# vressegu/sdeflow-light

Hardware: AMD Instinct MI355X
Metric: score-matching train steps/sec (+ reverse-SDE sample steps/sec) (higher is better)
Workload: dtype f32

## Files before the change

sdeflow_light_amd/csrc/conv_kernels.hip:

```cpp
#include "common.h"
#include <algorithm>
#include <type_traits>
#include <stdlib.h>

#define CONV_MAX_SRC 2

struct ConvGeom {
  int N, Hi, Wi, Ho, Wo;
  int KH, KW, strideH, padH, strideW, padW;
  int mode;
  int ups;
};

struct ConvArgs {
  ConvGeom g;
  const float* src[CONV_MAX_SRC];
  int C[CONV_MAX_SRC];
  int koff[CONV_MAX_SRC];
  int nsrc;
  const float* Wp;
  int Cout, CoutP, Ktot;
  const float* bias;
  const float* samp_bias;
  int n_bias, n_samp;
// ... 601 lines not shown
#pragma unroll
          for (int c = 0; c < 2; ++c) a[c] = *reinterpret_cast<const f32x4*>(wp + c * co_stride);
#pragma unroll
          for (int r = 0; r < 4; ++r)
#pragma unroll
            for (int c = 0; c < 2; ++c)
#pragma unroll
              for (int pt = 0; pt < 2; ++pt) acc[cls][c][pt] = mfma16(a[c][r], b[pt][r], acc[cls][c][pt]);
        }
      }
    }
  }
  asm volatile("s_nop 15\n\ts_nop 7" ::: "memory");
  __builtin_amdgcn_sched_barrier(0);
#pragma unroll
  for (int c = 0; c < 2; ++c) {
    const int co = co0 + 16 * c + 4 * q;
    const f32x4 add = conv_addend(A, n, co, true);
    f32x4 cs = {0.f, 0.f, 0.f, 0.f}, css = cs;
#pragma unroll
    for (int pt = 0; pt < 2; ++pt) {
      const int yy = y0 + 2 * w + pt, xx = x0 + il;
      if (yy >= g.Hi || xx >= g.Wi) continue;
#pragma unroll
      for (int cls = 0; cls < 4; ++cls) {
        const size_t m = ((size_t)n * g.Ho + 2 * yy + (cls >> 1)) * g.Wo + 2 * xx + (cls & 1);
        conv_store_quad(A, A.out + m * A.Cout + co, acc[cls][c][pt] + add, true, co, cs, css);
      }
    }
  }
}

#define C1_LP 36
template <int PT, int KG, int EXTRA>
__global__ void __launch_bounds__(256) k_conv1x1(ConvArgs A, int P , long Mtot, int ct_per) {
  constexpr bool LDS_OUT = PT == 4;
  __shared__ __attribute__((aligned(16))) float c1_lds[4][LDS_OUT ? 16 * PT * C1_LP : 4];
  const int tid = threadIdx.x, w = tid >> 6, lane = tid & 63, il = lane & 15, q = lane >> 4;
  const long m0 = ((long)blockIdx.x * 4 + w) * (16 * PT);
  if (m0 >= Mtot) return;
  float* wl = c1_lds[w];
  const int n = __builtin_amdgcn_readfirstlane((int)(m0 / P));
  const int g0 = A.C[0] >> 4;
  const int ctot = A.C[0] + (A.nsrc > 1 ? A.C[1] : 0);
  f32x4 b[PT][KG];
#pragma unroll
  for (int pt = 0; pt < PT; ++pt) {
    const long m = m0 + 16 * pt + il;
#pragma unroll
    for (int g = 0; g < KG; ++g) {
      const bool second = g >= g0;
      const int c = (second ? 16 * (g - g0) : 16 * g) + 4 * q;
      const int C = second ? A.C[1] : A.C[0];
      b[pt][g] = *reinterpret_cast<const f32x4*>((second ? A.src[1] : A.src[0]) + (size_t)m * C + c);
    }
  }
  if (A.in_scale) {
#pragma unroll
    for (int g = 0; g < KG; ++g) {
      const bool second = g >= g0;
      const size_t o = (size_t)n * ctot + (second ? A.C[0] + 16 * (g - g0) : 16 * g) + 4 * q;
      const f32x4 ga = *reinterpret_cast<const f32x4*>(A.in_scale + o), gb = *reinterpret_cast<const f32x4*>(A.in_shift + o);
#pragma unroll
      for (int pt = 0; pt < PT; ++pt) {
        f32x4 v = b[pt][g] * ga + gb;
        if (A.in_act == 1) {
#pragma unroll
          for (int r = 0; r < 4; ++r) v[r] = v[r] * __builtin_amdgcn_rcpf(1.0f + __expf(-v[r]));
        }
        b[pt][g] = v;
      }
    }
  }
  const int ct0 = blockIdx.y * ct_per, ntile = min(A.Cout >> 4, ct0 + ct_per);
  const float* wrow = A.Wp + (size_t)il * A.Ktot + 4 * q;
  const size_t tile_stride = (size_t)16 * A.Ktot;
  constexpr int D = (KG % 4 == 0) ? 4 : 2;
  static_assert(KG % D == 0 && D <= KG, "ring slots must line up from one tile to the next");
  f32x4 an[D];
#pragma unroll
  for (int d = 0; d < D; ++d) an[d] = *reinterpret_cast<const f32x4*>(wrow + (size_t)ct0 * tile_stride + 16 * d);
  const bool has_b = A.bias && n < A.n_bias, has_s = A.samp_bias && n < A.n_samp;
  const float fb = has_b ? 1.f : 0.f, fs = has_s ? 1.f : 0.f;
  const float* bp = has_b ? A.bias + 4 * q : A.Wp;
  const float* sp = has_s ? A.samp_bias + (size_t)n * A.Cout + 4 * q : A.Wp;
  const int bstep = has_b ? 16 : 0, sstep = has_s ? 16 : 0;
  f32x4 add_n = *reinterpret_cast<const f32x4*>(bp + (size_t)ct0 * bstep) * fb + *reinterpret_cast<const f32x4*>(sp + (size_t)ct0 * sstep) * fs;
  const float* ex = EXTRA ? (A.residual ? A.residual : A.out) : nullptr;
  const size_t orow = (size_t)(m0 + il) * A.Cout + 4 * q;
  const size_t ptstep = (size_t)16 * A.Cout;
  f32x4 ex_n[EXTRA ? PT : 1];
  if (EXTRA) {
#pragma unroll
    for (int pt = 0; pt < PT; ++pt) ex_n[pt] = *reinterpret_cast<const f32x4*>(ex + orow + pt * ptstep + 16 * ct0);
  }
  for (int ct = ct0; ct < ntile; ++ct) {
    const int ctn = min(ct + 1, ntile - 1);
    f32x4 acc[PT];
#pragma unroll
    for (int pt = 0; pt < PT; ++pt) acc[pt] = f32x4{0, 0, 0, 0};
    const f32x4 add = add_n;
    f32x4 exv[EXTRA ? PT : 1];
    if (EXTRA) {
#pragma unroll
      for (int pt = 0; pt < PT; ++pt) exv[pt] = ex_n[pt];
    }
#pragma unroll
    for (int g = 0; g < KG; ++g) {
      const f32x4 a = an[g % D];
      const int ng = (g + D < KG) ? g + D : g + D - KG, nct = (g + D < KG) ? ct : ctn;
      an[g % D] = *reinterpret_cast<const f32x4*>(wrow + (size_t)nct * tile_stride + 16 * ng);
      if (g == 0) {
        add_n = *reinterpret_cast<const f32x4*>(bp + (size_t)ctn * bstep) * fb + *reinterpret_cast<const f32x4*>(sp + (size_t)ctn * sstep) * fs;
        if (EXTRA) {
#pragma unroll
          for (int pt = 0; pt < PT; ++pt) ex_n[pt] = *reinterpret_cast<const f32x4*>(ex + orow + pt * ptstep + 16 * ctn);
        }
      }
      __builtin_amdgcn_sched_barrier(0);
#pragma unroll
      for (int r = 0; r < 4; ++r)
#pragma unroll
        for (int pt = 0; pt < PT; ++pt) acc[pt] = mfma16(a[r], b[pt][g][r], acc[pt]);
    }
    f32x4 cs = {0.f, 0.f, 0.f, 0.f}, css = {0.f, 0.f, 0.f, 0.f};
    const int half = (ct - ct0) & 1;
    const bool paired = LDS_OUT && (half == 1 || ct + 1 < ntile);
#pragma unroll
    for (int pt = 0; pt < PT; ++pt) {
      f32x4 v = acc[pt] + add;
      if (EXTRA) v += exv[pt];
      if (paired) *reinterpret_cast<f32x4*>(wl + (16 * pt + il) * C1_LP + 16 * half + 4 * q) = v;
      else *reinterpret_cast<f32x4*>(A.out + orow + pt * ptstep + 16 * ct) = v;
      cs += v; css += v * v;
    }
    if (LDS_OUT && half == 1) {
      const size_t obase = (size_t)m0 * A.Cout + 16 * (ct - 1) + 4 * (lane & 7);
#pragma unroll
      for (int j = 0; j < 2 * PT; ++j) {
        const int px = 8 * j + (lane >> 3);
        const f32x4 v = *reinterpret_cast<const f32x4*>(wl + px * C1_LP + 4 * (lane & 7));
        *reinterpret_cast<f32x4*>(A.out + obase + (size_t)px * A.Cout) = v;
        if (j & 1) __builtin_amdgcn_sched_barrier(0);
      }
    }
    if (A.cstat) cstat_store(A, n, (int)((m0 % P) / (16 * PT)), 16 * ct + 4 * q, cs, css, il);
  }
}

constexpr int H18_HW = 18, H18_ITEMS = H18_HW * H18_HW * (CT_KC / 4), H18_NST = (H18_ITEMS + 255) / 256;
__device__ __forceinline__ void halo18_load(const ConvArgs& A, const ConvGeom& g, const float* src, int C, int up, int c0, size_t aff0, int n, int y0, int x0,
                                            int tid, f32x4 (&st)[H18_NST], unsigned& valid, f32x4& ga, f32x4& gb) {
  const float* base = src + (size_t)n * g.Hi * g.Wi * C;
  const int cq = c0 + 4 * (tid & 7);
  ga = f32x4{1.f, 1.f, 1.f, 1.f}; gb = f32x4{0.f, 0.f, 0.f, 0.f};
  if (A.in_scale && cq < C) {
    const size_t o = aff0 + cq;
    ga = *reinterpret_cast<const f32x4*>(A.in_scale + o);
    gb = *reinterpret_cast<const f32x4*>(A.in_shift + o);
  }
  valid = 0;
#pragma unroll
  for (int k = 0; k < H18_NST; ++k) {
    const int idx = tid + 256 * k;
    f32x4 v = {0, 0, 0, 0};
    if (idx < H18_ITEMS) {
      const int hp = idx >> 3, hy = hp / H18_HW, hx = hp - hy * H18_HW;
      const int iy = y0 + hy - 1, ix = x0 + hx - 1;
      const int c = c0 + 4 * (idx & 7);
      if (iy >= 0 && iy < (g.Hi << up) && ix >= 0 && ix < (g.Wi << up) && c < C) {
        v = *reinterpret_cast<const f32x4*>(base + ((size_t)(iy >> up) * g.Wi + (ix >> up)) * C + c);
        valid |= 1u << k;
      }
    }
    st[k] = v;
  }
}
__device__ __forceinline__ void halo18_store(const ConvArgs& A, float* buf, int tid, f32x4 (&st)[H18_NST], unsigned valid, f32x4 ga, f32x4 gb) {
  if (A.in_scale) {
// ... 132 lines not shown
__device__ __forceinline__ void wino_patch_load(f32x4 (&d)[4][4], const float* __restrict__ p00, bool last_in_row) {
#pragma unroll
  for (int i = 0; i < 4; ++i) {
    d[i][0] = *reinterpret_cast<const f32x4*>(p00 + (i * HW_ + 0) * CT_P);
    d[i][1] = *reinterpret_cast<const f32x4*>(p00 + (i * HW_ + 1) * CT_P);
  }
#pragma unroll
  for (int i = 0; i < 4; ++i)
#pragma unroll
    for (int j = 0; j < 2; ++j)
#pragma unroll
      for (int r = 0; r < 4; ++r) d[i][2 + j][r] = dpp_from_next_lane(d[i][j][r]);
  if (last_in_row) {
#pragma unroll
    for (int i = 0; i < 4; ++i) {
      d[i][2] = *reinterpret_cast<const f32x4*>(p00 + (i * HW_ + 2) * CT_P);
      d[i][3] = *reinterpret_cast<const f32x4*>(p00 + (i * HW_ + 3) * CT_P);
    }
  }
}

__device__ __forceinline__ void wino_input_transform(f32x4 (&d)[4][4]) {
#pragma unroll
  for (int j = 0; j < 4; ++j) {
    const f32x4 r0 = d[0][j] - d[2][j], r1 = d[1][j] + d[2][j], r2 = d[2][j] - d[1][j], r3 = d[1][j] - d[3][j];
    d[0][j] = r0; d[1][j] = r1; d[2][j] = r2; d[3][j] = r3;
  }
#pragma unroll
  for (int i = 0; i < 4; ++i) {
    const f32x4 c0_ = d[i][0] - d[i][2], c1_ = d[i][1] + d[i][2], c2_ = d[i][2] - d[i][1], c3_ = d[i][1] - d[i][3];
    d[i][0] = c0_; d[i][1] = c1_; d[i][2] = c2_; d[i][3] = c3_;
  }
}
__device__ __forceinline__ void wino_wfill(const float* src, float* dst, int w, size_t pos_stride, size_t a_co_stride) {
#pragma unroll
  for (int j = 0; j < 4; ++j) {
    const int pw = 4 * w + j;
    __builtin_amdgcn_global_load_lds((const __attribute__((address_space(1))) void*)(src + (size_t)(pw >> 1) * pos_stride + (pw & 1) * a_co_stride),
                                     (__attribute__((address_space(3))) void*)(dst + pw * 256), 16, 0, 0);
  }
}
template <int NPOS>
__device__ __forceinline__ void wino_mfma_lds(f32x4 (&acc)[16][2], const f32x4 (&d)[4][4], const float* wb, int pos0) {
  f32x4 a0 = *reinterpret_cast<const f32x4*>(wb), a1 = *reinterpret_cast<const f32x4*>(wb + 256);
#pragma unroll
  for (int pl = 0; pl < NPOS; ++pl) {
    const f32x4 x0 = a0, x1 = a1;
    if (pl < NPOS - 1) {
      a0 = *reinterpret_cast<const f32x4*>(wb + (2 * pl + 2) * 256);
      a1 = *reinterpret_cast<const f32x4*>(wb + (2 * pl + 3) * 256);
    }
    const int pos = pos0 + pl;
    const f32x4 b = d[pos >> 2][pos & 3];
#pragma unroll
    for (int r = 0; r < 4; ++r) {
      acc[pos][0] = mfma16(x0[r], b[r], acc[pos][0]);
      acc[pos][1] = mfma16(x1[r], b[r], acc[pos][1]);
    }
    __builtin_amdgcn_sched_barrier(0);
  }
}

template <int NCO>
__device__ __forceinline__ void wino_output_transform(const f32x4 (&acc)[16][NCO], int c, f32x4 (&Y)[4]) {
  f32x4 t0[4], t1[4];
#pragma unroll
  for (int nu = 0; nu < 4; ++nu) {
    t0[nu] = acc[nu][c] + acc[4 + nu][c] + acc[8 + nu][c];
    t1[nu] = acc[4 + nu][c] - acc[8 + nu][c] - acc[12 + nu][c];
  }
// ... 266 lines not shown
  asm volatile("s_waitcnt vmcnt(0) lgkmcnt(0)\n\ts_barrier" ::: "memory");
  float* cur = hb0;
  float* nxt = hb1;
  const int ngrp = (C + 15) >> 4;
  for (; t < n_tiles; t += gridDim.x) {
    const int tn = t + gridDim.x;
    const bool more = tn < n_tiles;
    if (more) stage_load(tn);
    f32x4 acc[16][NCO];
#pragma unroll
    for (int p = 0; p < 16; ++p)
#pragma unroll
      for (int c = 0; c < NCO; ++c) acc[p][c] = f32x4{0, 0, 0, 0};
    for (int grp = 0; grp < ngrp; ++grp) {
      f32x4 d[4][4];
#pragma unroll
      for (int i = 0; i < 4; ++i)
#pragma unroll
        for (int j = 0; j < 4; ++j) d[i][j] = *reinterpret_cast<const f32x4*>(cur + pbase + (i * HW + j) * CT_P + 16 * grp);
      wino_input_transform(d);
      wino_mfma_lds<16>(acc, d, wbuf + grp * (16 * 2 * 256) + lane * 4, 0);
    }
    int n, y0, x0;
    tile_origin<16, 16>(t, tiles_x, tiles_y, n, y0, x0);
    wino_epilogue<NCO>(A, acc, n, y0, x0, w, 0, (t - n * tiles_x * tiles_y) * 4 + w, lane);
    if (more) halo18_store(A, nxt, tid, st, valid, ga, gb);
    asm volatile("s_waitcnt lgkmcnt(0)\n\ts_barrier" ::: "memory");
    float* sw = cur; cur = nxt; nxt = sw;
  }
}

constexpr int WP_HPIECES = 21;
constexpr int WP_HSTAGE = WP_HPIECES * 64 * 4;
constexpr int WP_LDS_BYTES = (2 * 4096 + 2 * WP_HSTAGE) * (int)sizeof(float);

__global__ void __launch_bounds__(256, 2) k_conv_wino_pipe(ConvArgs A, int tiles_x, int tiles_y, int n_tiles, int n_cob) {
  extern __shared__ __attribute__((aligned(16))) float cw_lds[];
  constexpr int NCO = 2, HW = 18;
  const int tid = threadIdx.x, lane = tid & 63, il = lane & 15, q = lane >> 4;
  const int w = __builtin_amdgcn_readfirstlane(tid >> 6);
  const ConvGeom g = A.g;
  float* wbuf = cw_lds;
  float* hbuf = cw_lds + 2 * 4096;
  const int xcd = blockIdx.x & 7, loc_stride = gridDim.x >> 3;
  int loc = blockIdx.x >> 3;
  int tile = (loc / n_cob) * 8 + xcd, cob = loc % n_cob;
  if (tile >= n_tiles) return;
  const int ngrp = A.Ktot >> 4, tpi = tiles_x * tiles_y, up = g.ups ? 1 : 0;
  const size_t a_co_stride = (size_t)16 * A.Ktot, pos_stride = (size_t)A.CoutP * A.Ktot;
  const int tt = 16 * w + il, ty = tt >> 3, tx = tt & 7;
  const int P0 = 2 * ty * HW + 2 * tx, h0 = (P0 >> 1) & 3;

  auto wfill = [&](int cob_, int grp_, int half) __attribute__((always_inline)) {
    wino_wfill(A.Wp + (size_t)(cob_ * (NCO * 16) + il) * A.Ktot + 16 * grp_ + 4 * q + (size_t)(8 * half) * pos_stride,
               wbuf + half * 4096, w, pos_stride, a_co_stride);
  };
  const int Hu = g.Hi << up, Wu = g.Wi << up;
  int hpk[(WP_HPIECES + 3) / 4];
#pragma unroll
  for (int j = 0; j < (WP_HPIECES + 3) / 4; ++j) {
    const int sl = 64 * (w + 4 * j) + lane, P = sl >> 2, c = (sl & 3) ^ ((P >> 1) & 3), hy = P / HW, hx = P - hy * HW;
    hpk[j] = P < HW * HW ? (hy << 16) | (hx << 2) | c : 0x7fff << 16;
  }
  auto hfill = [&](int tile_, int grp_, int b) __attribute__((always_inline)) {
    const int n = tile_ / tpi, r = tile_ - n * tpi, ty_i = r / tiles_x, y0 = ty_i * 16, x0 = (r - ty_i * tiles_x) * 16;
    const bool s1 = 16 * grp_ >= A.C[0];
    const int C = s1 ? A.C[1] : A.C[0];
    const float* base = (s1 ? A.src[1] : A.src[0]) + (size_t)n * g.Hi * g.Wi * C + (16 * grp_ - (s1 ? A.C[0] : 0));
#pragma unroll
    for (int j = 0; j < (WP_HPIECES + 3) / 4; ++j) {
      const int m = w + 4 * j;
      if (m < WP_HPIECES) {
        int pk = hpk[j];
        asm volatile("" : "+v"(pk));
        const int c = pk & 3, iy = y0 + (pk >> 16) - 1, ix = x0 + ((pk >> 2) & 31) - 1;
        const bool in = (unsigned)iy < (unsigned)Hu && (unsigned)ix < (unsigned)Wu;
        const float* p = in ? base + (((iy >> up) * g.Wi + (ix >> up)) * C + 4 * c) : g_wino_zero;
        __builtin_amdgcn_global_load_lds((const __attribute__((address_space(1))) void*)p,
                                         (__attribute__((address_space(3))) void*)(hbuf + b * WP_HSTAGE + m * 256), 16, 0, 0);
      }
    }
  };

  f32x4 acc[16][NCO];
#pragma unroll
  for (int p = 0; p < 16; ++p)
#pragma unroll
    for (int c = 0; c < NCO; ++c) acc[p][c] = f32x4{0, 0, 0, 0};
  int grp = 0, hb = 0;
  wfill(cob, 0, 0);
  hfill(tile, 0, 0);
  for (;;) {
    int nloc = loc, ntile = tile, ncob = cob, ngrp_ = grp + 1;
    if (ngrp_ == ngrp) {
      ngrp_ = 0; nloc = loc + loc_stride;
      ntile = (nloc / n_cob) * 8 + xcd; ncob = nloc % n_cob;
    }
    const bool more = ntile < n_tiles;
    f32x4 d[4][4];
#pragma unroll
    for (int half = 0; half < 2; ++half) {
      if (half == 1 && more) asm volatile("s_waitcnt vmcnt(5) lgkmcnt(0)\n\ts_barrier" ::: "memory");
      else asm volatile("s_waitcnt vmcnt(0) lgkmcnt(0)\n\ts_barrier" ::: "memory");
      if (half == 0) {
        wfill(cob, grp, 1);
        if (more) hfill(ntile, ngrp_, hb ^ 1);
      } else if (more) {
        wfill(ncob, ngrp_, 0);
      }
      if (half == 0) {
        const float* hs = hbuf + hb * WP_HSTAGE;
#pragma unroll
        for (int i = 0; i < 4; ++i) {
          const float* rp = hs + 16 * (P0 + i * HW) + 4 * (q ^ ((h0 + i) & 3));
          d[i][0] = *reinterpret_cast<const f32x4*>(rp);
          d[i][1] = *reinterpret_cast<const f32x4*>(rp + 16);
        }
#pragma unroll
        for (int i = 0; i < 4; ++i)
#pragma unroll
          for (int j = 0; j < 2; ++j)
#pragma unroll
            for (int r = 0; r < 4; ++r) d[i][2 + j][r] = dpp_from_next_lane(d[i][j][r]);
        if (tx == 7) {
#pragma unroll
          for (int i = 0; i < 4; ++i) {
            const float* rp = hs + 16 * (P0 + i * HW + 2) + 4 * (q ^ ((h0 + i + 1) & 3));
            d[i][2] = *reinterpret_cast<const f32x4*>(rp);
            d[i][3] = *reinterpret_cast<const f32x4*>(rp + 16);
          }
        }
        wino_input_transform(d);
      }
      const float* wb = wbuf + half * 4096 + lane * 4;
      f32x4 a0 = *reinterpret_cast<const f32x4*>(wb), a1 = *reinterpret_cast<const f32x4*>(wb + 256);
#pragma unroll
      for (int pl = 0; pl < 8; ++pl) {
        const f32x4 x0_ = a0, x1_ = a1;
        if (pl < 7) {
          a0 = *reinterpret_cast<const f32x4*>(wb + (2 * pl + 2) * 256);
          a1 = *reinterpret_cast<const f32x4*>(wb + (2 * pl + 3) * 256);
        }
        const int pos = 8 * half + pl;
        const f32x4 b = d[pos >> 2][pos & 3];
#pragma unroll
        for (int r = 0; r < 4; ++r) {
          acc[pos][0] = mfma16(x0_[r], b[r], acc[pos][0]);
          acc[pos][1] = mfma16(x1_[r], b[r], acc[pos][1]);
        }
        __builtin_amdgcn_sched_barrier(0);
      }
    }
    if (ngrp_ == 0) {
      const int n = tile / tpi, r = tile - n * tpi, ty_i = r / tiles_x;
      wino_epilogue<NCO>(A, acc, n, ty_i * 16, (r - ty_i * tiles_x) * 16, w, cob * (NCO * 16), r * 4 + w, lane);
      if (!more) break;
#pragma unroll
      for (int p = 0; p < 16; ++p)
#pragma unroll
        for (int c = 0; c < NCO; ++c) acc[p][c] = f32x4{0, 0, 0, 0};
    }
    loc = nloc; tile = ntile; cob = ncob; grp = ngrp_; hb ^= 1;
  }
}

__global__ void __launch_bounds__(256) k_wino_pack_batched(const msgm_pack_job_t* __restrict__ jobs) {
  const msgm_pack_job_t J = jobs[blockIdx.y];
  const int64_t tot = (int64_t)J.rows * J.ncols;
  for (int64_t e = blockIdx.x * (int64_t)blockDim.x + threadIdx.x; e < tot; e += (int64_t)gridDim.x * blockDim.x) {
    const int c = (int)(e % J.ncols), r = (int)(e / J.ncols);
    const float* w = J.W + r * J.sr + (J.col_off + c) * J.sc;
    float gk[3][3], h[4][3];
#pragma unroll
    for (int t = 0; t < 9; ++t) gk[t / 3][t % 3] = w[t * J.st];
#pragma unroll
    for (int j = 0; j < 3; ++j) {
      h[0][j] = gk[0][j];
      h[1][j] = 0.5f * (gk[0][j] + gk[1][j] + gk[2][j]);
      h[2][j] = 0.5f * (gk[0][j] - gk[1][j] + gk[2][j]);
      h[3][j] = gk[2][j];
    }
#pragma unroll
    for (int i = 0; i < 4; ++i) {
      const float u0 = h[i][0], u1 = 0.5f * (h[i][0] + h[i][1] + h[i][2]), u2 = 0.5f * (h[i][0] - h[i][1] + h[i][2]), u3 = h[i][2];
      float* p = J.Wp + ((int64_t)(4 * i) * J.rowsP + r) * J.Ktot + J.kp_off + c;
      const int64_t ps = (int64_t)J.rowsP * J.Ktot;
      p[0] = u0; p[ps] = u1; p[2 * ps] = u2; p[3 * ps] = u3;
    }
  }
}

struct WgradArgs {
  ConvGeom g;
  const float* gy;
  const float* src;
// ... 1026 lines not shown
}
static bool conv_has_masks(const ConvArgs& A) {
  unsigned m = 0;
  for (int i = 0; i < 16; ++i) m |= A.tapmask_in[i];
  for (int i = 0; i < 8; ++i) m |= A.tapmask_out[i];
  return m != 0;
}

int msgm_wino_pack_weights_batched(const msgm_pack_job_t* jobs, int32_t n_jobs, msgm_stream_t stream) {
  if (!jobs || n_jobs <= 0) return MSGM_E_BADARG;
  hipLaunchKernelGGL(k_wino_pack_batched, dim3(8, (unsigned)n_jobs), dim3(256), 0, S(stream), jobs);
  return msgm_check_launch();
}

static bool tile16_chanstats(ConvArgs& A) {
  if (!A.cstat) return true;
  A.cs_S = (A.g.Wo / 16) * (A.g.Ho / 16) * 4;
  return A.Cout % 4 == 0;
}

int msgm_conv_forward_wino(const msgm_conv_geom_t* geom, const float* src0, int32_t C0, const float* src1, int32_t C1,
                           const float* WpW, int32_t Cout, int32_t CoutP, int32_t Ktot, const float* bias,
                           const float* samp_bias, int32_t n_bias, int32_t n_samp, float* out, int32_t accumulate,
                           const msgm_conv_fuse_t* fuse, msgm_stream_t stream) {
  ConvArgs A;
  int rc = conv_args(&A, geom, src0, C0, src1, C1, WpW, Cout, CoutP, Ktot, bias, samp_bias, n_bias, n_samp, out, accumulate,
                     fuse, true);
  if (rc) return rc;
  if (!conv_wino_eligible(geom, C0, A.C[1], CoutP, 16) || !tile16_chanstats(A)) return MSGM_E_UNSUPPORTED;
  const int tiles_x = geom->Wo / 16, tiles_y = geom->Ho / 16;
  const int n_tiles = tiles_x * tiles_y * geom->N, gy = CoutP / 32;
  if (!A.in_scale) {
    conv_raise_lds_limit<&k_conv_wino_pipe, WP_LDS_BYTES>();
    const int items_per_xcd = gy * ((n_tiles + 7) / 8);
    const int wg_per_xcd = std::min(items_per_xcd, std::max(1, 2 * conv_n_cu() / 8));
    hipLaunchKernelGGL(k_conv_wino_pipe, dim3((unsigned)(8 * wg_per_xcd)), dim3(256), WP_LDS_BYTES, S(stream), A, tiles_x, tiles_y, n_tiles, gy);
    return msgm_check_launch();
  }
  const size_t lds = (size_t)18 * 18 * CT_P * sizeof(float);
  dim3 grid((unsigned)(8 * gy * ((n_tiles + 7) / 8)));
  constexpr int p32_min = 1024;
  if (!src1 && Ktot == 32 && CoutP == 32 && n_tiles >= p32_min) {
    conv_raise_lds_limit<&k_conv_wino_p32>();
    const size_t lds32 = ((size_t)2 * 16 * 2 * 256 + 2 * 18 * 18 * CT_P) * sizeof(float);
    hipLaunchKernelGGL(k_conv_wino_p32, dim3((unsigned)conv_n_cu()), dim3(256), lds32, S(stream), A, tiles_x, tiles_y, n_tiles);
    return msgm_check_launch();
  }
  if (Ktot < 64) {
    hipLaunchKernelGGL((k_conv_wino<2, false>), grid, dim3(256), lds, S(stream), A, tiles_x, tiles_y, n_tiles, gy);
    return msgm_check_launch();
  }
  conv_raise_lds_limit<&k_conv_wino<2, true>>();
  hipLaunchKernelGGL((k_conv_wino<2, true>), grid, dim3(256), lds + 2 * 4096 * sizeof(float), S(stream), A, tiles_x, tiles_y, n_tiles, gy);
  return msgm_check_launch();
}

__global__ void __launch_bounds__(256) k_b6_split(const float* __restrict__ Wp, __bf16* __restrict__ Wb, long n) {
  for (long e = (long)blockIdx.x * 256 + threadIdx.x; e < n; e += (long)gridDim.x * 256) {
    const float x = Wp[e];
    const __bf16 h = (__bf16)x;
    const float r1 = x - (float)h;
    const __bf16 m = (__bf16)r1;
    Wb[e] = h; Wb[n + e] = m; Wb[2 * n + e] = (__bf16)(r1 - (float)m);
  }
}

int msgm_conv_b6_supported(const msgm_conv_geom_t* geom, int32_t C0, int32_t C1, int32_t CoutP) {
  if (check_geom(geom)) return 0;
  return conv_wino_eligible(geom, C0, C1, CoutP, 32) ? 1 : 0;
// ... 3 lines not shown
  if (!Wp || !Wb || n_elem <= 0) return MSGM_E_BADARG;
  hipLaunchKernelGGL(k_b6_split, dim3((unsigned)grid_for(n_elem, 256, 2048)), dim3(256), 0, S(stream), Wp, static_cast<__bf16*>(Wb), (long)n_elem);
  return msgm_check_launch();
}

int msgm_conv_forward_b6(const msgm_conv_geom_t* geom, const float* src0, int32_t C0, const float* src1, int32_t C1,
                         const void* Wb, int32_t Cout, int32_t CoutP, int32_t Ktot, const float* bias,
                         const float* samp_bias, int32_t n_bias, int32_t n_samp, float* out, int32_t accumulate,
                         const msgm_conv_fuse_t* fuse, msgm_stream_t stream) {
  ConvArgs A;
  int rc = conv_args(&A, geom, src0, C0, src1, C1, Wb, Cout, CoutP, Ktot, bias, samp_bias, n_bias, n_samp, out, accumulate,
                     fuse, false);
  if (rc) return rc;
  if (!conv_wino_eligible(geom, C0, A.C[1], CoutP, 32) || conv_has_masks(A) || !tile16_chanstats(A)) return MSGM_E_UNSUPPORTED;
  const int nco = (CoutP % 64 == 0) ? 4 : 2;
  const int tiles_x = (geom->Wo + 15) / 16, tiles_y = (geom->Ho + 15) / 16;
  const int n_tiles = tiles_x * tiles_y * geom->N, gy = CoutP / (16 * nco);
  int per = (int)(((int64_t)n_tiles * gy) / (512 * 8));
  if (per > 4) per = 4;
  if (per < 1) per = 1;
  const int n_tgrp = (n_tiles + per - 1) / per;
  dim3 grid((unsigned)(8 * gy * ((n_tgrp + 7) / 8)));
  const size_t lds = (size_t)18 * 18 * 52 * sizeof(float);
  conv_raise_lds_limit<&k_conv_tile<16, 16, 4, 3, 4, false, true>>();
  conv_raise_lds_limit<&k_conv_tile<16, 16, 2, 3, 4, false, true>>();
  if (nco == 4) hipLaunchKernelGGL((k_conv_tile<16, 16, 4, 3, 4, false, true>), grid, dim3(256), lds, S(stream), A, 0, tiles_x, tiles_y, per, n_tiles, gy, n_tgrp);
  else hipLaunchKernelGGL((k_conv_tile<16, 16, 2, 3, 4, false, true>), grid, dim3(256), lds, S(stream), A, 0, tiles_x, tiles_y, per, n_tiles, gy, n_tgrp);
  return msgm_check_launch();
}

struct ConvRoute {
  int kind;
  int pt, kg;
  bool wide, two_d; int nco, TH, TW, tiles_x, tiles_y;
};
static bool conv_small_shape(const msgm_conv_geom_t* geom, bool has1, bool masks) {
  return conv_same(geom) && geom->KH == 3 && geom->KW == 3 && !geom->ups && geom->Ho > 1 && !has1 && !masks;
}
static bool conv_dgrad_s2_shape(const msgm_conv_geom_t* geom, int32_t C0, bool has1, int32_t Cout, int32_t CoutP, bool masks) {
  return geom->mode == 1 && geom->KH == 3 && geom->KW == 3 && geom->strideH == 2 && geom->strideW == 2 && geom->padH == 1 &&
         geom->padW == 1 && !geom->ups && geom->Ho == 2 * geom->Hi && geom->Wo == 2 * geom->Wi && !has1 && !masks &&
         C0 % 32 == 0 && Cout % 32 == 0 && CoutP == Cout;
}
static ConvRoute conv_route(const msgm_conv_geom_t* geom, int32_t C0, bool has1, int32_t C1, int32_t Cout, int32_t CoutP,
                            bool masks, bool both_extra = false , bool any_size = false) {
  ConvRoute r{};
  const int64_t Mtot = (int64_t)geom->N * geom->Ho * geom->Wo;
  if (conv_dgrad_s2_shape(geom, C0, has1, Cout, CoutP, masks)) { r.kind = 5; return r; }
  if (conv_small_shape(geom, has1, masks)) {
    if (C0 <= 4 && Cout == 32 && CoutP == 32) { r.kind = 3; return r; }
    if (C0 == 32 && Cout <= 4 && geom->mode == 0) { r.kind = 4; return r; }
  }
  const bool fast = (C0 % 16 == 0) && (!has1 || C1 % 16 == 0);
  const int Ktot = ((C0 + 15) / 16) * 16 + (has1 ? ((C1 + 15) / 16) * 16 : 0);
  const int kg = Ktot / 16;
  if (conv_same(geom) && geom->KH == 1 && geom->KW == 1 && !geom->ups && fast && !masks && (Mtot >= 4096 || any_size) &&
      (kg == 2 || kg == 4 || kg == 6 || kg == 8 || kg == 12 || kg == 16) && Cout % 16 == 0 && !both_extra) {
    const int pt = kg <= 4 ? 4 : (kg <= 8 ? 2 : (kg == 12 && (geom->Ho * geom->Wo) % 32 == 0 ? 2 : 1));
    if ((geom->Ho * geom->Wo) % (16 * pt) == 0) { r.kind = 1; r.kg = kg; r.pt = pt; return r; }
  }
  if (conv_tile_eligible(geom, C0, has1, C1, CoutP)) {
    r.kind = 2;
    r.two_d = geom->Ho > 1;
    r.nco = (CoutP % 64 == 0) ? 4 : 2;
    bool wide = geom->KW == 3 && (r.two_d ? (geom->Ho >= 16 && geom->Wo >= 16) : geom->Wo >= 256);
    if (wide) {
      const int64_t wtiles = (int64_t)geom->N * ((geom->Wo + (r.two_d ? 15 : 255)) / (r.two_d ? 16 : 256)) *
                             (r.two_d ? (geom->Ho + 15) / 16 : 1) * (CoutP / (16 * r.nco));
      if (wtiles < 512) wide = false;
    }
    r.wide = wide;
    r.TH = r.two_d ? (wide ? 16 : 8) : 1; r.TW = r.two_d ? 16 : (wide ? 256 : 128);
    r.tiles_x = (geom->Wo + r.TW - 1) / r.TW; r.tiles_y = (geom->Ho + r.TH - 1) / r.TH;
    if (!wide && r.nco == 4 && !masks && (int64_t)geom->N * r.tiles_x * r.tiles_y * (CoutP / 64) < 512) r.nco = 2;
    return r;
  }
  r.pt = (CoutP >= 64 && CoutP % 64 == 0) ? 2 : 4;
  return r;
}
static int conv_route_slots(const ConvRoute& r, const msgm_conv_geom_t* geom, int32_t Cout) {
  if (Cout % 4) return 0;
  if (r.kind == 1) { const int P = geom->Ho * geom->Wo; return P % (16 * r.pt) == 0 ? P / (16 * r.pt) : 0; }
  if (r.kind == 2) return r.tiles_x * r.tiles_y * 4;
  if (r.kind == 3) { const int P = geom->Ho * geom->Wo; return P % 64 == 0 ? P / 64 : 0; }
  if (r.kind == 4 || r.kind == 5) return 0;
  const int P = geom->Ho * geom->Wo, px = 16 * r.pt;
  return P % px == 0 ? P / px : 0;
}

int32_t msgm_conv_chanstats_slots(const msgm_conv_geom_t* geom, int32_t C0, int32_t C1, int32_t Cout, int32_t CoutP) {
  if (check_geom(geom) || C0 <= 0 || C1 < 0 || Cout <= 0 || CoutP < Cout || CoutP % 16) return 0;
  return conv_route_slots(conv_route(geom, C0, C1 > 0, C1, Cout, CoutP, false), geom, Cout);
// ... 43 lines not shown
    if (A.cs_S == 0 || A.cs_S != msgm_conv_chanstats_slots(geom, C0, src1 ? C1 : 0, Cout, CoutP)) return MSGM_E_UNSUPPORTED;
  }
  if (rt.kind == 3) {
    hipLaunchKernelGGL((k_conv3x3_cin_small<32>), dim3((unsigned)((Mtot + 255) / 256)), dim3(256), 0, S(stream), A, (long)Mtot);
    return msgm_check_launch();
  }
  if (rt.kind == 4) {
    const int tiles_x = (geom->Wo + 15) / 16, tiles_y = (geom->Ho + 15) / 16;
    const dim3 grid((unsigned)(tiles_x * tiles_y * geom->N));
    const size_t lds = (size_t)18 * 18 * CT_P * sizeof(float);
    switch (Cout) {
      case 1: hipLaunchKernelGGL((k_conv3x3_cout_small<1>), grid, dim3(256), lds, S(stream), A, tiles_x, tiles_y); break;
      case 2: hipLaunchKernelGGL((k_conv3x3_cout_small<2>), grid, dim3(256), lds, S(stream), A, tiles_x, tiles_y); break;
      case 3: hipLaunchKernelGGL((k_conv3x3_cout_small<3>), grid, dim3(256), lds, S(stream), A, tiles_x, tiles_y); break;
      default: hipLaunchKernelGGL((k_conv3x3_cout_small<4>), grid, dim3(256), lds, S(stream), A, tiles_x, tiles_y); break;
    }
    return msgm_check_launch();
  }
  if (rt.kind == 5) {
    const int tiles_x = (geom->Wi + DS_TW - 1) / DS_TW, tiles_y = (geom->Hi + DS_TH - 1) / DS_TH, n_cob = Cout / 32;
    const int64_t wgs = (int64_t)geom->N * tiles_x * tiles_y * n_cob;
    if (wgs >= (1ll << 31)) return MSGM_E_UNSUPPORTED;
    hipLaunchKernelGGL(k_dgrad_s2, dim3((unsigned)wgs), dim3(256), 0, S(stream), A, tiles_x, tiles_y, n_cob);
    return msgm_check_launch();
  }
  if (rt.kind == 1) {
    const int P = geom->Ho * geom->Wo;
    const int ntile = (Cout + 15) / 16;
    const long wgs = (Mtot + 64 * rt.pt - 1) / (64 * rt.pt);
    int split = wgs >= 768 ? 1 : (int)((768 + wgs - 1) / wgs);
    if (split > ntile) split = ntile;
    const int ct_per = (ntile + split - 1) / split, gy = (ntile + ct_per - 1) / ct_per;
    const bool extra = accumulate || A.residual;
#define C1_LAUNCH(PT_, KG_)                                                                                          \
  do {                                                                                                               \
    if (extra) hipLaunchKernelGGL((k_conv1x1<PT_, KG_, 1>), dim3((unsigned)wgs, (unsigned)gy), dim3(256), 0, S(stream), A, P, (long)Mtot, ct_per); \
    else hipLaunchKernelGGL((k_conv1x1<PT_, KG_, 0>), dim3((unsigned)wgs, (unsigned)gy), dim3(256), 0, S(stream), A, P, (long)Mtot, ct_per); \
  } while (0)
    switch (rt.kg) {
      case 2: C1_LAUNCH(4, 2); break;
      case 4: C1_LAUNCH(4, 4); break;
      case 6: C1_LAUNCH(2, 6); break;
      case 8: C1_LAUNCH(2, 8); break;
      case 12: if (rt.pt == 2) C1_LAUNCH(2, 12); else C1_LAUNCH(1, 12); break;
      default: C1_LAUNCH(1, 16); break;
    }
#undef C1_LAUNCH
    return msgm_check_launch();
  }
  if (rt.kind == 2) {
    const bool two_d = rt.two_d, wide = rt.wide;
    const int nco = rt.nco, TH = rt.TH, TW = rt.TW, tiles_x = rt.tiles_x, tiles_y = rt.tiles_y;
    const int halo = (TH + geom->KH - 1) * (TW + geom->KW - 1);
    const size_t lds = (size_t)(wide ? 1 : 2) * halo * CT_P * sizeof(float);
    const int n_tiles = tiles_x * tiles_y * geom->N, gy = CoutP / (16 * nco);
    constexpr int max_per = 4, rounds = 8;
    int per = (int)(((int64_t)n_tiles * gy) / (768 * rounds));
    if (per > max_per) per = max_per;
    if (per < 1) per = 1;
    const int n_tgrp = (n_tiles + per - 1) / per;
    dim3 grid((unsigned)(8 * gy * ((n_tgrp + 7) / 8)));
    const int flip = geom->mode;
#define CT_LAUNCH(TH_, TW_, NCO_, KS_, PT_, DB_) \
  hipLaunchKernelGGL((k_conv_tile<TH_, TW_, NCO_, KS_, PT_, DB_>), grid, dim3(256), lds, S(stream), A, flip, tiles_x, tiles_y, per, n_tiles, gy, n_tgrp)
    const bool k3 = geom->KW == 3;
    if (two_d) {
      if (wide) { if (nco == 4) CT_LAUNCH(16, 16, 4, 3, 4, false); else CT_LAUNCH(16, 16, 2, 3, 4, false); }
      else if (nco == 4) { if (k3) CT_LAUNCH(8, 16, 4, 3, 2, true); else CT_LAUNCH(8, 16, 4, 1, 2, true); }
      else { if (k3) CT_LAUNCH(8, 16, 2, 3, 2, true); else CT_LAUNCH(8, 16, 2, 1, 2, true); }
    } else {
// ... 353 lines not shown
```

Before: 10.25.

## Share Winograd weight tiles across two-tile teams in a 512-thread pipelined conv block

The pipelined Winograd conv kernel now runs 512-thread blocks made of two 4-wave teams. Each team works on a different spatial tile while sharing one double-buffered weight stage in LDS, and both teams cooperate to fill that stage. Halo address precomputation moves to a per-tile hitem step, and the halo loads are interleaved into the MFMA loop so they overlap compute. The intent is to halve weight LDS traffic and fills per output tile while keeping one block per CU. The cost is added complexity: an idle team keeps helping with weight fills, and the barrier and waitcnt logic becomes more intricate.

```diff
diff --git a/sdeflow_light_amd/csrc/conv_kernels.hip b/sdeflow_light_amd/csrc/conv_kernels.hip
--- a/sdeflow_light_amd/csrc/conv_kernels.hip
+++ b/sdeflow_light_amd/csrc/conv_kernels.hip
@@ -968,10 +968,11 @@
     d[i][0] = c0_; d[i][1] = c1_; d[i][2] = c2_; d[i][3] = c3_;
   }
 }
+template <int NW = 4>
 __device__ __forceinline__ void wino_wfill(const float* src, float* dst, int w, size_t pos_stride, size_t a_co_stride) {
 #pragma unroll
-  for (int j = 0; j < 4; ++j) {
-    const int pw = 4 * w + j;
+  for (int j = 0; j < 16 / NW; ++j) {
+    const int pw = (16 / NW) * w + j;
     __builtin_amdgcn_global_load_lds((const __attribute__((address_space(1))) void*)(src + (size_t)(pw >> 1) * pos_stride + (pw & 1) * a_co_stride),
                                      (__attribute__((address_space(3))) void*)(dst + pw * 256), 16, 0, 0);
   }
@@ -1304,53 +1305,60 @@
 
 constexpr int WP_HPIECES = 21;
 constexpr int WP_HSTAGE = WP_HPIECES * 64 * 4;
-constexpr int WP_LDS_BYTES = (2 * 4096 + 2 * WP_HSTAGE) * (int)sizeof(float);
-
-__global__ void __launch_bounds__(256, 2) k_conv_wino_pipe(ConvArgs A, int tiles_x, int tiles_y, int n_tiles, int n_cob) {
+constexpr int WP_TEAMS = 2;
+constexpr int WP_LDS_BYTES = (2 * 4096 + WP_TEAMS * 2 * WP_HSTAGE) * (int)sizeof(float);
+
+__global__ void __launch_bounds__(256 * WP_TEAMS, 1) k_conv_wino_pipe(ConvArgs A, int tiles_x, int tiles_y, int n_tiles, int n_cob, int tpu) {
   extern __shared__ __attribute__((aligned(16))) float cw_lds[];
-  constexpr int NCO = 2, HW = 18;
+  constexpr int NCO = 2, HW = 18, TEAMS = WP_TEAMS;
   const int tid = threadIdx.x, lane = tid & 63, il = lane & 15, q = lane >> 4;
-  const int w = __builtin_amdgcn_readfirstlane(tid >> 6);
+  const int w8 = __builtin_amdgcn_readfirstlane(tid >> 6), w = w8 & 3, team = w8 >> 2;
   const ConvGeom g = A.g;
   float* wbuf = cw_lds;
-  float* hbuf = cw_lds + 2 * 4096;
+  float* hbuf = cw_lds + 2 * 4096 + team * 2 * WP_HSTAGE;
   const int xcd = blockIdx.x & 7, loc_stride = gridDim.x >> 3;
+  const int n_units = (n_tiles + tpu - 1) / tpu;
   int loc = blockIdx.x >> 3;
-  int tile = (loc / n_cob) * 8 + xcd, cob = loc % n_cob;
-  if (tile >= n_tiles) return;
+  int unit = (loc / n_cob) * 8 + xcd, cob = loc % n_cob;
+  if (unit >= n_units) return;
   const int ngrp = A.Ktot >> 4, tpi = tiles_x * tiles_y, up = g.ups ? 1 : 0;
   const size_t a_co_stride = (size_t)16 * A.Ktot, pos_stride = (size_t)A.CoutP * A.Ktot;
   const int tt = 16 * w + il, ty = tt >> 3, tx = tt & 7;
   const int P0 = 2 * ty * HW + 2 * tx, h0 = (P0 >> 1) & 3;
 
   auto wfill = [&](int cob_, int grp_, int half) __attribute__((always_inline)) {
-    wino_wfill(A.Wp + (size_t)(cob_ * (NCO * 16) + il) * A.Ktot + 16 * grp_ + 4 * q + (size_t)(8 * half) * pos_stride,
-               wbuf + half * 4096, w, pos_stride, a_co_stride);
+    wino_wfill<4 * TEAMS>(A.Wp + (size_t)(cob_ * (NCO * 16) + il) * A.Ktot + 16 * grp_ + 4 * q + (size_t)(8 * half) * pos_stride,
+                          wbuf + half * 4096, w8, pos_stride, a_co_stride);
   };
   const int Hu = g.Hi << up, Wu = g.Wi << up;
-  int hpk[(WP_HPIECES + 3) / 4];
-#pragma unroll
-  for (int j = 0; j < (WP_HPIECES + 3) / 4; ++j) {
-    const int sl = 64 * (w + 4 * j) + lane, P = sl >> 2, c = (sl & 3) ^ ((P >> 1) & 3), hy = P / HW, hx = P - hy * HW;
-    hpk[j] = P < HW * HW ? (hy << 16) | (hx << 2) | c : 0x7fff << 16;
-  }
-  auto hfill = [&](int tile_, int grp_, int b) __attribute__((always_inline)) {
+  int hpk[(WP_HPIECES + 3) / 4], hn = 0;
+  auto hitem = [&](int tile_) __attribute__((always_inline)) {
     const int n = tile_ / tpi, r = tile_ - n * tpi, ty_i = r / tiles_x, y0 = ty_i * 16, x0 = (r - ty_i * tiles_x) * 16;
+    hn = n;
+    int l = lane;
+    asm volatile("" : "+v"(l));
+#pragma unroll
+    for (int j = 0; j < (WP_HPIECES + 3) / 4; ++j) {
+      const int sl = 64 * (w + 4 * j) + l, P = sl >> 2, c = (sl & 3) ^ ((P >> 1) & 3), hy = P / HW, hx = P - hy * HW;
+      const int iy = y0 + hy - 1, ix = x0 + hx - 1;
+      const bool in = tile_ >= 0 && P < HW * HW && (unsigned)iy < (unsigned)Hu && (unsigned)ix < (unsigned)Wu;
+      hpk[j] = in ? (((iy >> up) * g.Wi + (ix >> up)) << 2) | c : -1;
+    }
+  };
+  auto hsrc = [&](int grp_, int& C) __attribute__((always_inline)) {
     const bool s1 = 16 * grp_ >= A.C[0];
-    const int C = s1 ? A.C[1] : A.C[0];
-    const float* base = (s1 ? A.src[1] : A.src[0]) + (size_t)n * g.Hi * g.Wi * C + (16 * grp_ - (s1 ? A.C[0] : 0));
-#pragma unroll
-    for (int j = 0; j < (WP_HPIECES + 3) / 4; ++j) {
-      const int m = w + 4 * j;
-      if (m < WP_HPIECES) {
-        int pk = hpk[j];
-        asm volatile("" : "+v"(pk));
-        const int c = pk & 3, iy = y0 + (pk >> 16) - 1, ix = x0 + ((pk >> 2) & 31) - 1;
-        const bool in = (unsigned)iy < (unsigned)Hu && (unsigned)ix < (unsigned)Wu;
-        const float* p = in ? base + (((iy >> up) * g.Wi + (ix >> up)) * C + 4 * c) : g_wino_zero;
-        __builtin_amdgcn_global_load_lds((const __attribute__((address_space(1))) void*)p,
-                                         (__attribute__((address_space(3))) void*)(hbuf + b * WP_HSTAGE + m * 256), 16, 0, 0);
-      }
+    C = s1 ? A.C[1] : A.C[0];
+    return (s1 ? A.src[1] : A.src[0]) + (size_t)hn * g.Hi * g.Wi * C + (16 * grp_ - (s1 ? A.C[0] : 0));
+  };
+  auto hpiece = [&](int j, const float* base, int C, int b) __attribute__((always_inline)) {
+    const int m = w + 4 * j;
+    if (m < WP_HPIECES) {
+      const int pk = hpk[j];
+      const bool in = pk >= 0;
+      const unsigned off = in ? (unsigned)((pk >> 2) * C + 4 * (pk & 3)) : 0u;
+      const float* p = (in ? base : (const float*)g_wino_zero) + off;
+      __builtin_amdgcn_global_load_lds((const __attribute__((address_space(1))) void*)p,
+                                       (__attribute__((address_space(3))) void*)(hbuf + b * WP_HSTAGE + m * 256), 16, 0, 0);
     }
   };
 
@@ -1361,22 +1369,34 @@
     for (int c = 0; c < NCO; ++c) acc[p][c] = f32x4{0, 0, 0, 0};
   int grp = 0, hb = 0;
   wfill(cob, 0, 0);
-  hfill(tile, 0, 0);
-  for (;;) {
-    int nloc = loc, ntile = tile, ncob = cob, ngrp_ = grp + 1;
+  const bool lone = team >= tpu || tpu * unit + team >= n_tiles;
+  if (!lone) {
+    hitem(tpu * unit + team);
+    int C;
+    const float* base = hsrc(0, C);
+#pragma unroll
+    for (int j = 0; j < (WP_HPIECES + 3) / 4; ++j) hpiece(j, base, C, 0);
+  }
+  while (!lone) {
+    int nloc = loc, nunit = unit, ncob = cob, ngrp_ = grp + 1;
     if (ngrp_ == ngrp) {
       ngrp_ = 0; nloc = loc + loc_stride;
-      ntile = (nloc / n_cob) * 8 + xcd; ncob = nloc % n_cob;
-    }
-    const bool more = ntile < n_tiles;
+      nunit = (nloc / n_cob) * 8 + xcd; ncob = nloc % n_cob;
+    }
+    const bool more = nunit < n_units;
+    const int ntile = tpu * nunit + team;
+    const bool nact = more && ntile < n_tiles;
     f32x4 d[4][4];
 #pragma unroll
     for (int half = 0; half < 2; ++half) {
-      if (half == 1 && more) asm volatile("s_waitcnt vmcnt(5) lgkmcnt(0)\n\ts_barrier" ::: "memory");
+      if (half == 1) asm volatile("s_waitcnt vmcnt(5) lgkmcnt(0)\n\ts_barrier" ::: "memory");
       else asm volatile("s_waitcnt vmcnt(0) lgkmcnt(0)\n\ts_barrier" ::: "memory");
+      int hC = 0;
+      const float* hbase = nullptr;
       if (half == 0) {
         wfill(cob, grp, 1);
-        if (more) hfill(ntile, ngrp_, hb ^ 1);
+        if (nunit != unit) hitem(nact ? ntile : -1);
+        hbase = hsrc(ngrp_, hC);
       } else if (more) {
         wfill(ncob, ngrp_, 0);
       }
@@ -1420,19 +1440,42 @@
           acc[pos][0] = mfma16(x0_[r], b[r], acc[pos][0]);
           acc[pos][1] = mfma16(x1_[r], b[r], acc[pos][1]);
         }
+        if (half == 0 && pl < (WP_HPIECES + 3) / 4) hpiece(pl, hbase, hC, hb ^ 1);
         __builtin_amdgcn_sched_barrier(0);
       }
     }
     if (ngrp_ == 0) {
-      const int n = tile / tpi, r = tile - n * tpi, ty_i = r / tiles_x;
+      const int tile = tpu * unit + team, n = tile / tpi, r = tile - n * tpi, ty_i = r / tiles_x;
       wino_epilogue<NCO>(A, acc, n, ty_i * 16, (r - ty_i * tiles_x) * 16, w, cob * (NCO * 16), r * 4 + w, lane);
-      if (!more) break;
+      if (!nact) {
+        if (!more) {
+          asm volatile("s_waitcnt vmcnt(0)" ::: "memory");
+          return;
+        }
+        loc = nloc; cob = ncob;
+        break;
+      }
 #pragma unroll
       for (int p = 0; p < 16; ++p)
 #pragma unroll
         for (int c = 0; c < NCO; ++c) acc[p][c] = f32x4{0, 0, 0, 0};
     }
-    loc = nloc; tile = ntile; cob = ncob; grp = ngrp_; hb ^= 1;
+    loc = nloc; unit = nunit; cob = ncob; grp = ngrp_; hb ^= 1;
+  }
+  {
+    for (grp = 0;; ++grp) {
+      const bool last = grp + 1 == ngrp;
+      const int nloc = loc + loc_stride;
+      const bool more = !last || (nloc / n_cob) * 8 + xcd < n_units;
+      asm volatile("s_waitcnt vmcnt(0) lgkmcnt(0)\n\ts_barrier" ::: "memory");
+      wfill(cob, grp, 1);
+      asm volatile("s_waitcnt vmcnt(0) lgkmcnt(0)\n\ts_barrier" ::: "memory");
+      if (!more) return;
+      if (last) {
+        loc = nloc; cob = nloc % n_cob; grp = -1;
+      }
+      wfill(cob, grp + 1, 0);
+    }
   }
 }
 
@@ -2525,9 +2568,11 @@
   const int n_tiles = tiles_x * tiles_y * geom->N, gy = CoutP / 32;
   if (!A.in_scale) {
     conv_raise_lds_limit<&k_conv_wino_pipe, WP_LDS_BYTES>();
-    const int items_per_xcd = gy * ((n_tiles + 7) / 8);
-    const int wg_per_xcd = std::min(items_per_xcd, std::max(1, 2 * conv_n_cu() / 8));
-    hipLaunchKernelGGL(k_conv_wino_pipe, dim3((unsigned)(8 * wg_per_xcd)), dim3(256), WP_LDS_BYTES, S(stream), A, tiles_x, tiles_y, n_tiles, gy);
+    const int cu_per_xcd = std::max(1, conv_n_cu() / 8);
+    const int tpu = gy * ((n_tiles + 7) / 8) > cu_per_xcd ? 2 : 1;
+    const int items_per_xcd = gy * (((n_tiles + tpu - 1) / tpu + 7) / 8);
+    const int wg_per_xcd = std::min(items_per_xcd, cu_per_xcd);
+    hipLaunchKernelGGL(k_conv_wino_pipe, dim3((unsigned)(8 * wg_per_xcd)), dim3(256 * WP_TEAMS), WP_LDS_BYTES, S(stream), A, tiles_x, tiles_y, n_tiles, gy, tpu);
     return msgm_check_launch();
   }
   const size_t lds = (size_t)18 * 18 * CT_P * sizeof(float);
```

New measurement: 10.32, median of 6. No clear change (+0.7%).

## Stage 1x1 conv weights in LDS and loop persistent tiles per workgroup

Applied to the files above, without the earlier changes.

Adds a weight-in-LDS variant of the 1x1 conv kernel. The workgroup's weight slice is copied once into shared memory with global_load_lds, bias plus per-sample bias is precomputed into a per-wave strip, and each workgroup then loops over several pixel tiles so the staged weights are reused. The goal is to stop re-reading weights and bias from global memory for every tile. The price is more LDS per workgroup, which can lower occupancy, plus a barrier on the first tile and more complex grid sizing. The paired-store LDS buffer is also shrunk by writing half-tiles in two passes.

```diff
diff --git a/sdeflow_light_amd/csrc/conv_kernels.hip b/sdeflow_light_amd/csrc/conv_kernels.hip
--- a/sdeflow_light_amd/csrc/conv_kernels.hip
+++ b/sdeflow_light_amd/csrc/conv_kernels.hip
@@ -657,14 +657,10 @@
 }
 
 #define C1_LP 36
-template <int PT, int KG, int EXTRA>
-__global__ void __launch_bounds__(256) k_conv1x1(ConvArgs A, int P , long Mtot, int ct_per) {
+template <int PT, int KG, int EXTRA, bool WL>
+__device__ __forceinline__ void conv1x1_wave_tile(const ConvArgs& A, int P, long m0, int lane, float* wl, float* strip, const float* wimg, int ct0, int ntile, bool meet) {
   constexpr bool LDS_OUT = PT == 4;
-  __shared__ __attribute__((aligned(16))) float c1_lds[4][LDS_OUT ? 16 * PT * C1_LP : 4];
-  const int tid = threadIdx.x, w = tid >> 6, lane = tid & 63, il = lane & 15, q = lane >> 4;
-  const long m0 = ((long)blockIdx.x * 4 + w) * (16 * PT);
-  if (m0 >= Mtot) return;
-  float* wl = c1_lds[w];
+  const int il = lane & 15, q = lane >> 4;
   const int n = __builtin_amdgcn_readfirstlane((int)(m0 / P));
   const int g0 = A.C[0] >> 4;
   const int ctot = A.C[0] + (A.nsrc > 1 ? A.C[1] : 0);
@@ -680,6 +676,9 @@
       b[pt][g] = *reinterpret_cast<const f32x4*>((second ? A.src[1] : A.src[0]) + (size_t)m * C + c);
     }
   }
+  if constexpr (WL) {
+    if (meet) asm volatile("s_waitcnt vmcnt(0)\n\ts_barrier" ::: "memory");
+  }
   if (A.in_scale) {
 #pragma unroll
     for (int g = 0; g < KG; ++g) {
@@ -697,20 +696,34 @@
       }
     }
   }
-  const int ct0 = blockIdx.y * ct_per, ntile = min(A.Cout >> 4, ct0 + ct_per);
   const float* wrow = A.Wp + (size_t)il * A.Ktot + 4 * q;
   const size_t tile_stride = (size_t)16 * A.Ktot;
+  auto wfrag = [&](int ct, int g) __attribute__((always_inline)) {
+    if constexpr (WL) return *reinterpret_cast<const f32x4*>(wimg + ((ct - ct0) * KG + g) * 256 + 4 * lane);
+    else return *reinterpret_cast<const f32x4*>(wrow + (size_t)ct * tile_stride + 16 * g);
+  };
   constexpr int D = (KG % 4 == 0) ? 4 : 2;
   static_assert(KG % D == 0 && D <= KG, "ring slots must line up from one tile to the next");
   f32x4 an[D];
 #pragma unroll
-  for (int d = 0; d < D; ++d) an[d] = *reinterpret_cast<const f32x4*>(wrow + (size_t)ct0 * tile_stride + 16 * d);
+  for (int d = 0; d < D; ++d) an[d] = wfrag(ct0, d);
   const bool has_b = A.bias && n < A.n_bias, has_s = A.samp_bias && n < A.n_samp;
   const float fb = has_b ? 1.f : 0.f, fs = has_s ? 1.f : 0.f;
   const float* bp = has_b ? A.bias + 4 * q : A.Wp;
   const float* sp = has_s ? A.samp_bias + (size_t)n * A.Cout + 4 * q : A.Wp;
   const int bstep = has_b ? 16 : 0, sstep = has_s ? 16 : 0;
-  f32x4 add_n = *reinterpret_cast<const f32x4*>(bp + (size_t)ct0 * bstep) * fb + *reinterpret_cast<const f32x4*>(sp + (size_t)ct0 * sstep) * fs;
+  if constexpr (WL) {
+    for (int i = lane; i < 4 * (ntile - ct0); i += 64) {
+      const int c = 16 * ct0 + 4 * i;
+      const f32x4 vb = *reinterpret_cast<const f32x4*>(has_b ? A.bias + c : A.Wp), vs = *reinterpret_cast<const f32x4*>(has_s ? A.samp_bias + (size_t)n * A.Cout + c : A.Wp);
+      *reinterpret_cast<f32x4*>(strip + 4 * i) = vb * fb + vs * fs;
+    }
+  }
+  auto addend = [&](int ct) __attribute__((always_inline)) {
+    if constexpr (WL) return *reinterpret_cast<const f32x4*>(strip + 16 * (ct - ct0) + 4 * q);
+    else return *reinterpret_cast<const f32x4*>(bp + (size_t)ct * bstep) * fb + *reinterpret_cast<const f32x4*>(sp + (size_t)ct * sstep) * fs;
+  };
+  f32x4 add_n = addend(ct0);
   const float* ex = EXTRA ? (A.residual ? A.residual : A.out) : nullptr;
   const size_t orow = (size_t)(m0 + il) * A.Cout + 4 * q;
   const size_t ptstep = (size_t)16 * A.Cout;
@@ -719,6 +732,7 @@
 #pragma unroll
     for (int pt = 0; pt < PT; ++pt) ex_n[pt] = *reinterpret_cast<const f32x4*>(ex + orow + pt * ptstep + 16 * ct0);
   }
+  f32x4 vprev[WL && LDS_OUT ? PT : 1];
   for (int ct = ct0; ct < ntile; ++ct) {
     const int ctn = min(ct + 1, ntile - 1);
     f32x4 acc[PT];
@@ -734,9 +748,9 @@
     for (int g = 0; g < KG; ++g) {
       const f32x4 a = an[g % D];
       const int ng = (g + D < KG) ? g + D : g + D - KG, nct = (g + D < KG) ? ct : ctn;
-      an[g % D] = *reinterpret_cast<const f32x4*>(wrow + (size_t)nct * tile_stride + 16 * ng);
+      an[g % D] = wfrag(nct, ng);
       if (g == 0) {
-        add_n = *reinterpret_cast<const f32x4*>(bp + (size_t)ctn * bstep) * fb + *reinterpret_cast<const f32x4*>(sp + (size_t)ctn * sstep) * fs;
+        add_n = addend(ctn);
         if (EXTRA) {
 #pragma unroll
           for (int pt = 0; pt < PT; ++pt) ex_n[pt] = *reinterpret_cast<const f32x4*>(ex + orow + pt * ptstep + 16 * ctn);
@@ -751,14 +765,42 @@
     f32x4 cs = {0.f, 0.f, 0.f, 0.f}, css = {0.f, 0.f, 0.f, 0.f};
     const int half = (ct - ct0) & 1;
     const bool paired = LDS_OUT && (half == 1 || ct + 1 < ntile);
+    f32x4 vcur[WL && LDS_OUT ? PT : 1];
 #pragma unroll
     for (int pt = 0; pt < PT; ++pt) {
       f32x4 v = acc[pt] + add;
       if (EXTRA) v += exv[pt];
-      if (paired) *reinterpret_cast<f32x4*>(wl + (16 * pt + il) * C1_LP + 16 * half + 4 * q) = v;
-      else *reinterpret_cast<f32x4*>(A.out + orow + pt * ptstep + 16 * ct) = v;
+      if constexpr (WL && LDS_OUT) {
+        if (!paired) *reinterpret_cast<f32x4*>(A.out + orow + pt * ptstep + 16 * ct) = v;
+        else if (half == 0) vprev[pt] = v;
+        vcur[pt] = v;
+      } else {
+        if (paired) *reinterpret_cast<f32x4*>(wl + (16 * pt + il) * C1_LP + 16 * half + 4 * q) = v;
+        else *reinterpret_cast<f32x4*>(A.out + orow + pt * ptstep + 16 * ct) = v;
+      }
       cs += v; css += v * v;
     }
+    if constexpr (WL && LDS_OUT) {
+      if (half == 1) {
+        const size_t obase = (size_t)m0 * A.Cout + 16 * (ct - 1) + 4 * (lane & 7);
+#pragma unroll
+        for (int h = 0; h < PT / 2; ++h) {
+#pragma unroll
+          for (int k = 0; k < 2; ++k) {
+            float* wp = wl + (16 * k + il) * C1_LP + 4 * q;
+            *reinterpret_cast<f32x4*>(wp) = vprev[2 * h + k];
+            *reinterpret_cast<f32x4*>(wp + 16) = vcur[2 * h + k];
+          }
+#pragma unroll
+          for (int j = 0; j < 4; ++j) {
+            const int px = 8 * j + (lane >> 3);
+            const f32x4 v = *reinterpret_cast<const f32x4*>(wl + px * C1_LP + 4 * (lane & 7));
+            *reinterpret_cast<f32x4*>(A.out + obase + (size_t)(32 * h + px) * A.Cout) = v;
+            if (j & 1) __builtin_amdgcn_sched_barrier(0);
+          }
+        }
+      }
+    } else
     if (LDS_OUT && half == 1) {
       const size_t obase = (size_t)m0 * A.Cout + 16 * (ct - 1) + 4 * (lane & 7);
 #pragma unroll
@@ -770,6 +812,33 @@
       }
     }
     if (A.cstat) cstat_store(A, n, (int)((m0 % P) / (16 * PT)), 16 * ct + 4 * q, cs, css, il);
+  }
+}
+template <int PT, int KG, int EXTRA, bool WL = false>
+__global__ void __launch_bounds__(256) k_conv1x1(ConvArgs A, int P , long Mtot, int ct_per, int per) {
+  constexpr int C1W = PT == 4 ? (WL ? 32 : 16 * PT) * C1_LP : 4;
+  __shared__ __attribute__((aligned(16))) float c1_lds[4][WL ? 4 : C1W];
+  const int tid = threadIdx.x, w = tid >> 6, lane = tid & 63;
+  const int ct0 = blockIdx.y * ct_per, ntile = min(A.Cout >> 4, ct0 + ct_per);
+  if constexpr (WL) {
+    extern __shared__ __attribute__((aligned(16))) float c1_wimg[];
+    const float* wsrc = A.Wp + (size_t)(16 * ct0 + (lane & 15)) * A.Ktot + 4 * (lane >> 4);
+    const int npiece = (ntile - ct0) * KG;
+    for (int p = w; p < npiece; p += 4) {
+      const int ctl = p / KG, g = p - ctl * KG;
+      __builtin_amdgcn_global_load_lds((const __attribute__((address_space(1))) void*)(wsrc + (size_t)ctl * (16 * A.Ktot) + 16 * g),
+                                       (__attribute__((address_space(3))) void*)(c1_wimg + p * 256), 16, 0, 0);
+    }
+    for (int t = 0; t < per; ++t) {
+      const long m0 = (((long)blockIdx.x * per + t) * 4 + w) * (16 * PT);
+      float* priv = c1_wimg + ct_per * (KG * 256) + w * (C1W + 16 * ct_per);
+      if (m0 < Mtot) conv1x1_wave_tile<PT, KG, EXTRA, true>(A, P, m0, lane, priv, priv + C1W, c1_wimg, ct0, ntile, t == 0);
+      else if (t == 0) asm volatile("s_waitcnt vmcnt(0)\n\ts_barrier" ::: "memory");
+    }
+  } else {
+    const long m0 = ((long)blockIdx.x * 4 + w) * (16 * PT);
+    if (m0 >= Mtot) return;
+    conv1x1_wave_tile<PT, KG, EXTRA, false>(A, P, m0, lane, c1_lds[w], nullptr, nullptr, ct0, ntile, false);
   }
 }
 
@@ -2597,6 +2666,7 @@
 struct ConvRoute {
   int kind;
   int pt, kg;
+  bool wl;
   bool wide, two_d; int nco, TH, TW, tiles_x, tiles_y;
 };
 static bool conv_small_shape(const msgm_conv_geom_t* geom, bool has1, bool masks) {
@@ -2622,7 +2692,7 @@
   if (conv_same(geom) && geom->KH == 1 && geom->KW == 1 && !geom->ups && fast && !masks && (Mtot >= 4096 || any_size) &&
       (kg == 2 || kg == 4 || kg == 6 || kg == 8 || kg == 12 || kg == 16) && Cout % 16 == 0 && !both_extra) {
     const int pt = kg <= 4 ? 4 : (kg <= 8 ? 2 : (kg == 12 && (geom->Ho * geom->Wo) % 32 == 0 ? 2 : 1));
-    if ((geom->Ho * geom->Wo) % (16 * pt) == 0) { r.kind = 1; r.kg = kg; r.pt = pt; return r; }
+    if ((geom->Ho * geom->Wo) % (16 * pt) == 0) { r.kind = 1; r.kg = kg; r.pt = pt; r.wl = kg >= 4 && kg <= 12; return r; }
   }
   if (conv_tile_eligible(geom, C0, has1, C1, CoutP)) {
     r.kind = 2;
@@ -2732,10 +2802,37 @@
     if (split > ntile) split = ntile;
     const int ct_per = (ntile + split - 1) / split, gy = (ntile + ct_per - 1) / ct_per;
     const bool extra = accumulate || A.residual;
+    const int cap = 64 / rt.kg;
+    const int ct_wl = ct_per < cap ? ct_per : cap, gy_wl = (ntile + ct_wl - 1) / ct_wl;
+    if (rt.wl && gy_wl <= (gy > 2 ? gy : 2)) {
+      const size_t lds = (size_t)ct_wl * rt.kg * 1024 + 4 * ((rt.pt == 4 ? (size_t)32 * C1_LP : 4) + 16 * ct_wl) * sizeof(float);
+      long occ = (long)(160 * 1024 / lds);
+      if (occ > 4) occ = 4;
+      const long slots = occ * conv_n_cu();
+      const long r8 = gy_wl > 1 ? 8 : 1;
+      int per = (int)((wgs * gy_wl + slots - 1) / slots);
+      long wgs_wl = ((wgs + per - 1) / per + r8 - 1) / r8 * r8;
+      while (per > 1 && wgs_wl * gy_wl > slots) { ++per; wgs_wl = ((wgs + per - 1) / per + r8 - 1) / r8 * r8; }
+#define C1_LAUNCH_WL(PT_, KG_)                                                                                       \
+  do {                                                                                                               \
+    conv_raise_lds_limit<&k_conv1x1<PT_, KG_, 0, true>>();                                                           \
+    conv_raise_lds_limit<&k_conv1x1<PT_, KG_, 1, true>>();                                                           \
+    if (extra) hipLaunchKernelGGL((k_conv1x1<PT_, KG_, 1, true>), dim3((unsigned)wgs_wl, (unsigned)gy_wl), dim3(256), lds, S(stream), A, P, (long)Mtot, ct_wl, per); \
+    else hipLaunchKernelGGL((k_conv1x1<PT_, KG_, 0, true>), dim3((unsigned)wgs_wl, (unsigned)gy_wl), dim3(256), lds, S(stream), A, P, (long)Mtot, ct_wl, per); \
+  } while (0)
+      switch (rt.kg) {
+        case 4: C1_LAUNCH_WL(4, 4); break;
+        case 6: C1_LAUNCH_WL(2, 6); break;
+        case 8: C1_LAUNCH_WL(2, 8); break;
+        default: if (rt.pt == 2) C1_LAUNCH_WL(2, 12); else C1_LAUNCH_WL(1, 12); break;
+      }
+#undef C1_LAUNCH_WL
+      return msgm_check_launch();
+    }
 #define C1_LAUNCH(PT_, KG_)                                                                                          \
   do {                                                                                                               \
-    if (extra) hipLaunchKernelGGL((k_conv1x1<PT_, KG_, 1>), dim3((unsigned)wgs, (unsigned)gy), dim3(256), 0, S(stream), A, P, (long)Mtot, ct_per); \
-    else hipLaunchKernelGGL((k_conv1x1<PT_, KG_, 0>), dim3((unsigned)wgs, (unsigned)gy), dim3(256), 0, S(stream), A, P, (long)Mtot, ct_per); \
+    if (extra) hipLaunchKernelGGL((k_conv1x1<PT_, KG_, 1>), dim3((unsigned)wgs, (unsigned)gy), dim3(256), 0, S(stream), A, P, (long)Mtot, ct_per, 1); \
+    else hipLaunchKernelGGL((k_conv1x1<PT_, KG_, 0>), dim3((unsigned)wgs, (unsigned)gy), dim3(256), 0, S(stream), A, P, (long)Mtot, ct_per, 1); \
   } while (0)
     switch (rt.kg) {
       case 2: C1_LAUNCH(4, 2); break;
```

After: 10.23 before, 10.27 after (median of 6 runs). No clear change (+0.4%).
